# thuanz123/enhancing-transformers

Hardware: AMD Instinct MI355X
Metric: images/sec ViT-VQGAN-base 256px stage-1 train; VQ argmin match-rate (higher is better)
Workload: dtype fp16; 1 GPU; imagenet_vitvq_base.yaml AE training step (1 fwd + 1 bwd + grad all-reduce + AdamW), loss = 1.0*L2 + 1.0*codebook (LPIPS/GAN weights 0), K=8192 x 32 l2-normalised codes, fp32 master weights, fp16 MFMA operands / fp32 accumulate, dynamic loss scale (now 65536; device-side inf/nan step skip + GradScaler update rule); per_gpu_batch=128, global_batch=128, image=256x256, parallelism=dp1, hip_graph_replay=False

## Files before the change

### enhancing-transformers_amd/csrc/common.h

```cpp
#pragma once
#include <hip/hip_runtime.h>
#include <stdint.h>
#include <stdio.h>
#include "../../include/enh_hip.h"

#define LDS_AS __attribute__((address_space(3)))
#define GLB_AS __attribute__((address_space(1)))
#ifdef ENH_GLDS_AUX_OVERRIDE
#define ENH_GLDS_AUX ENH_GLDS_AUX_OVERRIDE
#else
#define ENH_GLDS_AUX 0
#endif

typedef __attribute__((ext_vector_type(4))) float f32x4;
typedef __attribute__((ext_vector_type(4))) unsigned int u32x4;
typedef __attribute__((ext_vector_type(2))) unsigned int u32x2;
typedef __attribute__((ext_vector_type(16))) float f32x16;
typedef __attribute__((ext_vector_type(8))) __bf16 bf16x8;
typedef __attribute__((ext_vector_type(8))) short s16x8;
typedef __attribute__((ext_vector_type(4))) short s16x4;
typedef __attribute__((__vector_size__(4 * sizeof(__bf16)))) __bf16 bf16x4_t;

void enh_set_error(const char* fmt, ...);
int enh_check_launch(const char* what);
// ... 49 lines not shown
  else return (float)__builtin_bit_cast(f16x2_t, u)[1];
}
template <typename OT>
__device__ inline float unpack1(uint16_t h) {
  if constexpr (OT::id == 0) return __builtin_bit_cast(float, (uint32_t)h << 16);
  else return (float)__builtin_bit_cast(_Float16, h);
}
template <typename OT>
__device__ inline uint16_t pack1(float f) {
  if constexpr (OT::id == 0) return f32_to_bf16_bits(f);
  else return __builtin_bit_cast(uint16_t, (_Float16)f);
}
template <typename OT>
__device__ __forceinline__ f32x16 mfma32(const s16x8& a, const s16x8& b, const f32x16& c) {
  if constexpr (OT::id == 0) return __builtin_amdgcn_mfma_f32_32x32x16_bf16(__builtin_bit_cast(bf16x8, a), __builtin_bit_cast(bf16x8, b), c, 0, 0, 0);
  else return __builtin_amdgcn_mfma_f32_32x32x16_f16(__builtin_bit_cast(f16x8, a), __builtin_bit_cast(f16x8, b), c, 0, 0, 0);
}
template <typename OT>
__device__ __forceinline__ f32x4 mfma16(const s16x8& a, const s16x8& b, const f32x4& c) {
  if constexpr (OT::id == 0) return __builtin_amdgcn_mfma_f32_16x16x32_bf16(__builtin_bit_cast(bf16x8, a), __builtin_bit_cast(bf16x8, b), c, 0, 0, 0);
  else return __builtin_amdgcn_mfma_f32_16x16x32_f16(__builtin_bit_cast(f16x8, a), __builtin_bit_cast(f16x8, b), c, 0, 0, 0);
}
#define ENH_DT_DISPATCH(dtype, CALL)                    \
  do {                                                   \
    if ((dtype) == ENH_DT_F16) { typedef F16 OT; CALL; } \
    else { typedef BF16 OT; CALL; }                      \
  } while (0)
#define ENH_REQUIRE_DT(dtype, what) ENH_REQUIRE((dtype) == ENH_DT_BF16 || (dtype) == ENH_DT_F16, ENH_E_BADARG, what ": dtype must be ENH_DT_BF16 (0) or ENH_DT_F16 (1), got %d", (int)(dtype))

__device__ __forceinline__ float tanh_x3(float x) {
  const float x2 = x * x;
  const float t = __builtin_amdgcn_exp2f(x * 2.8853900817779268f);
  const float big = 1.f - 2.f * __builtin_amdgcn_rcpf(t + 1.f);
  const float small = x * (1.f + x2 * (-0.33333333333f + x2 * (0.13333333333f + x2 * -0.05396825397f)));
  return x2 < 0.0144f ? small : big;
}

__device__ inline s16x4 lds_tr_read_b64(const void* lds_ptr) {
  bf16x4_t v = __builtin_amdgcn_ds_read_tr16_b64_v4bf16((LDS_AS bf16x4_t*)lds_ptr);
  return __builtin_bit_cast(s16x4, v);
}

__device__ inline void lds_tr_read_b64_asm(unsigned long long& out, const void* lds_ptr) {
  const unsigned addr = (unsigned)(uintptr_t)(LDS_AS const void*)lds_ptr;
  asm volatile("ds_read_b64_tr_b16 %0, %1" : "=v"(out) : "v"(addr) : "memory");
}

__device__ inline float wave_sum(float v) {
#pragma unroll
  for (int o = 32; o > 0; o >>= 1) v += __shfl_xor(v, o, 64);
  return v;
}

__device__ inline float fixed_order_rowsum16(const float* __restrict__ part, int rows, int64_t stride, int64_t n, bool n_ok, float* s_red ) {
  const int col = threadIdx.x & 15, grp = threadIdx.x >> 4;
  const int per = (rows + 15) / 16;
  const int r0 = grp * per, r1 = r0 + per < rows ? r0 + per : rows;
  float a = 0.f;
  if (n_ok)
    for (int r = r0; r < r1; ++r) a += part[(int64_t)r * stride + n];
  s_red[grp * 16 + col] = a;
  __syncthreads();
  float t = 0.f;
  if (grp == 0)
    for (int g = 0; g < 16; ++g) t += s_red[g * 16 + col];
  return t;
}
```

### enhancing-transformers_amd/csrc/elementwise.hip

```cpp
#include "common.h"

template <typename OT>
__global__ void patchify_kernel(const float* __restrict__ img, int B, int C, int H, int W, int p,
                                uint16_t* __restrict__ out, int64_t total4) {
  const int64_t i = (int64_t)blockIdx.x * blockDim.x + threadIdx.x;
  if (i >= total4) return;
  const int p4 = p >> 2, gx_n = W / p, gy_n = H / p;
  int64_t r = i;
  const int q = (int)(r % p4); r /= p4;
  const int ph = (int)(r % p); r /= p;
  const int c = (int)(r % C); r /= C;
  const int gx = (int)(r % gx_n);
  const int gy = (int)((r / gx_n) % gy_n);
  const int b = (int)(r / ((int64_t)gx_n * gy_n));
  const float4 v = *reinterpret_cast<const float4*>(img + (((size_t)b * C + c) * H + (size_t)gy * p + ph) * W + (size_t)gx * p + q * 4);
  *reinterpret_cast<uint2*>(out + (size_t)i * 4) = make_uint2(pack2<OT>(v.x, v.y), pack2<OT>(v.z, v.w));
}

template <typename OT>
__global__ __launch_bounds__(256) void unpatchify_loss_kernel(
    const float* __restrict__ pix, const float* __restrict__ target, int B, int C, int H, int W, int p, float w_l1,
    float w_l2, float inv_numel, float* __restrict__ xrec, double* __restrict__ sums, uint16_t* __restrict__ dpix,
    int64_t total4, const float* __restrict__ gscale) {
  __shared__ float s_l1[4], s_l2[4];
  if (gscale) inv_numel *= *gscale;
  const int64_t i = (int64_t)blockIdx.x * blockDim.x + threadIdx.x;
  float l1 = 0.f, l2 = 0.f;
  if (i < total4) {
    const int p4 = p >> 2, gx_n = W / p, gy_n = H / p;
    int64_t r = i;
    const int q = (int)(r % p4); r /= p4;
    const int ph = (int)(r % p); r /= p;
    const int c = (int)(r % C); r /= C;
    const int gx = (int)(r % gx_n);
    const int gy = (int)((r / gx_n) % gy_n);
    const int b = (int)(r / ((int64_t)gx_n * gy_n));
    const size_t off = (((size_t)b * C + c) * H + (size_t)gy * p + ph) * W + (size_t)gx * p + q * 4;
    const float4 v = *reinterpret_cast<const float4*>(pix + (size_t)i * 4);
    if (xrec) *reinterpret_cast<float4*>(xrec + off) = v;
    if (target) {
      const float4 x = *reinterpret_cast<const float4*>(target + off);
      const float d[4] = {v.x - x.x, v.y - x.y, v.z - x.z, v.w - x.w};
      float g[4];
#pragma unroll
      for (int k = 0; k < 4; ++k) {
        l1 += fabsf(d[k]);
        l2 += d[k] * d[k];
        const float sg = d[k] > 0.f ? 1.f : (d[k] < 0.f ? -1.f : 0.f);
        g[k] = (w_l1 * sg + w_l2 * 2.f * d[k]) * inv_numel;
      }
      if (dpix) *reinterpret_cast<uint2*>(dpix + (size_t)i * 4) = make_uint2(pack2<OT>(g[0], g[1]), pack2<OT>(g[2], g[3]));
    }
  }
  if (sums) {
    l1 = wave_sum(l1);
    l2 = wave_sum(l2);
    if ((threadIdx.x & 63) == 0) { s_l1[threadIdx.x >> 6] = l1; s_l2[threadIdx.x >> 6] = l2; }
    __syncthreads();
    if (threadIdx.x == 0) {
      atomicAdd(&sums[0], (double)((s_l1[0] + s_l1[1]) + (s_l1[2] + s_l1[3])));
      atomicAdd(&sums[1], (double)((s_l2[0] + s_l2[1]) + (s_l2[2] + s_l2[3])));
    }
  }
}

template <typename OT>
__global__ __launch_bounds__(256) void colsum_h16_kernel(const uint16_t* __restrict__ x, int64_t M, int64_t N,
                                                          int64_t ldx, int64_t rows_per_block, float* __restrict__ out, int64_t part_stride) {
  __shared__ float s_part[3][128];
  const int lane = threadIdx.x & 63, wave = threadIdx.x >> 6;
  const int64_t n0 = (int64_t)blockIdx.x * 128 + lane * 2;
  const int64_t m_begin = (int64_t)blockIdx.y * rows_per_block;
  int64_t m_end = m_begin + rows_per_block;
  if (m_end > M) m_end = M;
  float a0 = 0.f, a1 = 0.f;
  if (n0 < N) {
    for (int64_t m = m_begin + wave; m < m_end; m += 4) {
      const uint32_t u = *reinterpret_cast<const uint32_t*>(x + (size_t)m * ldx + n0);
      a0 += unpack_lo<OT>(u);
      a1 += unpack_hi<OT>(u);
    }
  }
  if (wave > 0) { s_part[wave - 1][lane * 2] = a0; s_part[wave - 1][lane * 2 + 1] = a1; }
  __syncthreads();
  if (wave == 0 && n0 < N) {
    for (int ww = 0; ww < 3; ++ww) { a0 += s_part[ww][lane * 2]; a1 += s_part[ww][lane * 2 + 1]; }
    { if (part_stride) out[(int64_t)blockIdx.y * part_stride + n0] = a0; else atomicAdd(&out[n0], a0); }
    { if (part_stride) out[(int64_t)blockIdx.y * part_stride + n0 + 1] = a1; else atomicAdd(&out[n0 + 1], a1); }
  }
}

template <typename OT>
__global__ __launch_bounds__(256) void colsum_h16_wide_kernel(const uint16_t* __restrict__ x, int64_t M, int64_t N, int64_t ldx,
                                                               int64_t rows_per_block, float* __restrict__ out, int64_t part_stride) {
  __shared__ float s_part[3][512];
  const int lane = threadIdx.x & 63, wave = threadIdx.x >> 6;
  const int64_t n0 = (int64_t)blockIdx.x * 512 + lane * 8;
  const int64_t m_begin = (int64_t)blockIdx.y * rows_per_block;
  int64_t m_end = m_begin + rows_per_block;
  if (m_end > M) m_end = M;
  float acc[8] = {0.f, 0.f, 0.f, 0.f, 0.f, 0.f, 0.f, 0.f};
  if (n0 < N) {
    const uint16_t* col = x + n0;
    int64_t m = m_begin + wave;
    for (; m + 12 < m_end; m += 16) {
      u32x4 v[4];
#pragma unroll
      for (int r = 0; r < 4; ++r) v[r] = *reinterpret_cast<const u32x4*>(col + (size_t)(m + 4 * r) * ldx);
#pragma unroll
      for (int r = 0; r < 4; ++r)
#pragma unroll
        for (int k = 0; k < 4; ++k) {
          acc[2 * k] += unpack_lo<OT>(v[r][k]);
          acc[2 * k + 1] += unpack_hi<OT>(v[r][k]);
        }
// ... 42 lines not shown
  if (i >= n) return;
  if (skip && *skip != 0.f) return;
  if (loss_scale) gscale /= *loss_scale;
  float pv[4], gv[4], mv[4], vv[4];
  const bool full = i + 3 < n;
  if (full) {
    const float4 a = *reinterpret_cast<const float4*>(p + i), b = *reinterpret_cast<const float4*>(g + i);
    const float4 c = *reinterpret_cast<const float4*>(m + i), d = *reinterpret_cast<const float4*>(v + i);
    pv[0] = a.x; pv[1] = a.y; pv[2] = a.z; pv[3] = a.w; gv[0] = b.x; gv[1] = b.y; gv[2] = b.z; gv[3] = b.w;
    mv[0] = c.x; mv[1] = c.y; mv[2] = c.z; mv[3] = c.w; vv[0] = d.x; vv[1] = d.y; vv[2] = d.z; vv[3] = d.w;
  } else {
    for (int k = 0; k < 4; ++k) {
      const bool ok = i + k < n;
      pv[k] = ok ? p[i + k] : 0.f; gv[k] = ok ? g[i + k] : 0.f; mv[k] = ok ? m[i + k] : 0.f; vv[k] = ok ? v[i + k] : 0.f;
    }
  }
#pragma unroll
  for (int k = 0; k < 4; ++k) {
    const float gg = gv[k] * gscale;
    pv[k] = pv[k] * (1.0f - lr * wd);
    mv[k] = mv[k] * beta1 + gg * (1.0f - beta1);
    vv[k] = vv[k] * beta2 + gg * gg * (1.0f - beta2);
    const float denom = sqrtf(vv[k]) * inv_sqrt_bc2 + eps;
    pv[k] = pv[k] - (lr * inv_bc1) * (mv[k] / denom);
  }
  if (full) {
    *reinterpret_cast<float4*>(p + i) = make_float4(pv[0], pv[1], pv[2], pv[3]);
    *reinterpret_cast<float4*>(m + i) = make_float4(mv[0], mv[1], mv[2], mv[3]);
    *reinterpret_cast<float4*>(v + i) = make_float4(vv[0], vv[1], vv[2], vv[3]);
    if (p16) *reinterpret_cast<uint2*>(p16 + i) = make_uint2(pack2<OT>(pv[0], pv[1]), pack2<OT>(pv[2], pv[3]));
  } else {
    for (int k = 0; k < 4 && i + k < n; ++k) {
      p[i + k] = pv[k]; m[i + k] = mv[k]; v[i + k] = vv[k];
      if (p16) p16[i + k] = pack1<OT>(pv[k]);
    }
  }
}

extern "C" int enh_patchify(const float* img, int B, int C, int H, int W, int p, enh_h16* patches, int dtype, void* stream) {
  ENH_REQUIRE_DT(dtype, "enh_patchify");
  ENH_REQUIRE(img && patches, ENH_E_BADARG, "enh_patchify: null pointer");
  ENH_REQUIRE(B > 0 && C > 0 && p > 0 && p % 4 == 0 && H % p == 0 && W % p == 0, ENH_E_SHAPE, "enh_patchify: need p %% 4 == 0 and H,W divisible by p (B=%d C=%d H=%d W=%d p=%d)", B, C, H, W, p);
  const int64_t total4 = (int64_t)B * C * H * W / 4;
  ENH_DT_DISPATCH(dtype, (patchify_kernel<OT><<<(int)((total4 + 255) / 256), 256, 0, (hipStream_t)stream>>>(img, B, C, H, W, p, patches, total4)));
  return enh_check_launch("enh_patchify");
}

extern "C" int enh_unpatchify_loss(const float* pix, const float* target, int B, int C, int H, int W, int p, float w_l1,
                                   float w_l2, float* xrec, double* sums, enh_h16* dpix_bf16, const float* grad_scale_dev, int dtype, void* stream) {
  ENH_REQUIRE_DT(dtype, "enh_unpatchify_loss");
  ENH_REQUIRE(pix && (xrec || target), ENH_E_BADARG, "enh_unpatchify_loss: null pointer");
  ENH_REQUIRE(B > 0 && C > 0 && p > 0 && p % 4 == 0 && H % p == 0 && W % p == 0, ENH_E_SHAPE, "enh_unpatchify_loss: need p %% 4 == 0 and H,W divisible by p");
  const int64_t numel = (int64_t)B * C * H * W, total4 = numel / 4;
  ENH_DT_DISPATCH(dtype, (unpatchify_loss_kernel<OT><<<(int)((total4 + 255) / 256), 256, 0, (hipStream_t)stream>>>(
      pix, target, B, C, H, W, p, w_l1, w_l2, 1.0f / (float)numel, xrec, target ? sums : nullptr, dpix_bf16, total4, grad_scale_dev)));
  return enh_check_launch("enh_unpatchify_loss");
}

__global__ __launch_bounds__(256) void colsum_reduce_kernel(const float* __restrict__ part, int chunks, int64_t N, float* __restrict__ out, int accumulate) {
  __shared__ float s_red[256];
  const int64_t n = (int64_t)blockIdx.x * 16 + (threadIdx.x & 15);
  const float t = fixed_order_rowsum16(part, chunks, N, n, n < N, s_red);
  if ((threadIdx.x >> 4) == 0 && n < N) out[n] = accumulate ? out[n] + t : t;
}

int enh_colsum_reduce_launch(const float* part, int chunks, int64_t N, float* out, int accumulate, hipStream_t s) {
  colsum_reduce_kernel<<<dim3((unsigned)((N + 15) / 16)), 256, 0, s>>>(part, chunks, N, out, accumulate);
  return enh_check_launch("colsum_reduce");
}

static int64_t colsum_chunks(int64_t M) {
  const int64_t chunks = (M + 511) / 512;
  return chunks > 256 ? 256 : chunks;
}

extern "C" size_t enh_colsum_h16_workspace_bytes(int64_t M, int64_t N) { return M > 0 && N > 0 ? (size_t)colsum_chunks(M) * N * sizeof(float) : 0; }

static int colsum_h16_impl(const enh_h16* x, int64_t M, int64_t N, int64_t ldx, float* out, int accumulate, float* part, int dtype, void* stream) {
  ENH_REQUIRE_DT(dtype, "enh_colsum_h16");
  ENH_REQUIRE(x && out, ENH_E_BADARG, "enh_colsum_h16: null pointer");
  ENH_REQUIRE(M > 0 && N > 0 && N % 2 == 0 && ldx % 2 == 0, ENH_E_SHAPE, "enh_colsum_h16: N and ldx must be even");
  hipStream_t s = (hipStream_t)stream;
  if (!accumulate && !part) {
    const int rc = enh_zero_f32_launch(out, N, s);
    if (rc) return rc;
  }
  const int64_t chunks = colsum_chunks(M);
  const int64_t rows_per_block = (M + chunks - 1) / chunks;
  float* dst = part ? part : out;
  const int64_t stride = part ? N : 0;
  if (N % 8 == 0 && ldx % 8 == 0 && ((uintptr_t)x & 15) == 0) {
    dim3 grid((unsigned)((N + 511) / 512), (unsigned)chunks);
    ENH_DT_DISPATCH(dtype, (colsum_h16_wide_kernel<OT><<<grid, 256, 0, s>>>(x, M, N, ldx, rows_per_block, dst, stride)));
  } else {
    dim3 grid((unsigned)((N + 127) / 128), (unsigned)chunks);
    ENH_DT_DISPATCH(dtype, (colsum_h16_kernel<OT><<<grid, 256, 0, s>>>(x, M, N, ldx, rows_per_block, dst, stride)));
  }
  if (part) colsum_reduce_kernel<<<dim3((unsigned)((N + 15) / 16)), 256, 0, s>>>(part, (int)chunks, N, out, accumulate);
  return enh_check_launch("enh_colsum_h16");
}

extern "C" int enh_colsum_h16(const enh_h16* x, int64_t M, int64_t N, int64_t ldx, float* out, int accumulate, int dtype, void* stream) {
  return colsum_h16_impl(x, M, N, ldx, out, accumulate, nullptr, dtype, stream);
}

extern "C" int enh_colsum_h16_ws(const enh_h16* x, int64_t M, int64_t N, int64_t ldx, float* out, int accumulate, void* ws, size_t ws_bytes, int dtype, void* stream) {
  ENH_REQUIRE(ws && ws_bytes >= enh_colsum_h16_workspace_bytes(M, N), ENH_E_WORKSPACE, "enh_colsum_h16_ws: workspace too small (%zu bytes)", ws_bytes);
  return colsum_h16_impl(x, M, N, ldx, out, accumulate, (float*)ws, dtype, stream);
}

template <typename OT>
__global__ void cast_f32_h16_head_scaled_kernel(const float* __restrict__ x, uint16_t* __restrict__ y, int64_t n, int64_t n_scaled, float alpha,
                                                 int64_t x_stride, int64_t y_stride) {
  x += (int64_t)blockIdx.y * x_stride; y += (int64_t)blockIdx.y * y_stride;
  const int64_t i = ((int64_t)blockIdx.x * blockDim.x + threadIdx.x) * 4;
  if (i >= n) return;
  if (i + 3 < n) {
    float4 v = *reinterpret_cast<const float4*>(x + i);
    if (i < n_scaled) { v.x *= alpha; v.y *= alpha; v.z *= alpha; v.w *= alpha; }
    *reinterpret_cast<uint2*>(y + i) = make_uint2(pack2<OT>(v.x, v.y), pack2<OT>(v.z, v.w));
  } else {
    for (int64_t k = i; k < n; ++k) y[k] = pack1<OT>(x[k] * (k < n_scaled ? alpha : 1.0f));
  }
}

extern "C" int enh_cast_f32_h16_head_scaled(const float* x, enh_h16* y, int64_t n, int64_t n_scaled, float alpha, int dtype, void* stream) {
  ENH_REQUIRE_DT(dtype, "enh_cast_f32_h16_head_scaled");
  ENH_REQUIRE(x && y && n > 0 && n_scaled >= 0 && n_scaled <= n && n_scaled % 4 == 0, ENH_E_BADARG, "enh_cast_f32_h16_head_scaled: bad argument");
  const int64_t n4 = (n + 3) / 4;
  ENH_DT_DISPATCH(dtype, (cast_f32_h16_head_scaled_kernel<OT><<<(int)((n4 + 255) / 256), 256, 0, (hipStream_t)stream>>>(x, y, n, n_scaled, alpha, 0, 0)));
  return enh_check_launch("enh_cast_f32_h16_head_scaled");
}

extern "C" int enh_cast_f32_h16_head_scaled_strided(const float* x, int64_t x_stride, enh_h16* y, int64_t y_stride, int64_t n, int64_t n_scaled, float alpha,
                                                     int count, int dtype, void* stream) {
  ENH_REQUIRE_DT(dtype, "enh_cast_f32_h16_head_scaled_strided");
  ENH_REQUIRE(x && y && n > 0 && n_scaled >= 0 && n_scaled <= n && n_scaled % 4 == 0 && count > 0 && count <= 65535, ENH_E_BADARG,
              "enh_cast_f32_h16_head_scaled_strided: bad argument");
  ENH_REQUIRE(x_stride % 4 == 0 && y_stride % 4 == 0 && y_stride >= n, ENH_E_SHAPE, "enh_cast_f32_h16_head_scaled_strided: strides must be multiples of 4 elements and the outputs disjoint");
  const int64_t n4 = (n + 3) / 4;
  ENH_DT_DISPATCH(dtype, (cast_f32_h16_head_scaled_kernel<OT><<<dim3((unsigned)((n4 + 255) / 256), (unsigned)count), 256, 0, (hipStream_t)stream>>>(x, y, n, n_scaled, alpha, x_stride, y_stride)));
  return enh_check_launch("enh_cast_f32_h16_head_scaled_strided");
}

extern "C" int enh_cast_f32_h16(const float* x, enh_h16* y, int64_t n, int dtype, void* stream) {
  ENH_REQUIRE_DT(dtype, "enh_cast_f32_h16");
  ENH_REQUIRE(x && y && n > 0, ENH_E_BADARG, "enh_cast_f32_h16: bad argument");
  const int64_t n4 = (n + 3) / 4;
  ENH_DT_DISPATCH(dtype, (cast_f32_h16_kernel<OT><<<(int)((n4 + 255) / 256), 256, 0, (hipStream_t)stream>>>(x, y, n)));
  return enh_check_launch("enh_cast_f32_h16");
}
// ... 77 lines not shown
```

### enhancing-transformers_amd/csrc/layernorm.hip

```cpp
#include "common.h"

template <int NCH, bool X3, typename OT>
__global__ __launch_bounds__(256) void ln_fwd_kernel(const float* __restrict__ x, const float* __restrict__ w,
                                                     const float* __restrict__ b, int64_t M, int D, float eps,
                                                     uint16_t* __restrict__ y16, float* __restrict__ y32,
                                                     float* __restrict__ mean_out, float* __restrict__ rstd_out, uint16_t* __restrict__ y3) {
  const int lane = threadIdx.x & 63;
  const int64_t row = (int64_t)blockIdx.x * 4 + (threadIdx.x >> 6);
  if (row >= M) return;
  const int nch = D >> 2;
  const float4* xr = reinterpret_cast<const float4*>(x + (size_t)row * D);
  float4 v[NCH];
  float s = 0.f;
#pragma unroll
  for (int i = 0; i < NCH; ++i) {
    const int c = lane + 64 * i;
    v[i] = c < nch ? xr[c] : make_float4(0.f, 0.f, 0.f, 0.f);
    s += (v[i].x + v[i].y) + (v[i].z + v[i].w);
  }
  const float mean = wave_sum(s) / (float)D;
  float q = 0.f;
#pragma unroll
  for (int i = 0; i < NCH; ++i) {
    const int c = lane + 64 * i;
// ... 179 lines not shown
            for (int ww = 0; ww < 3; ++ww) ax[k] += s_dw[ww][c * 4 + k];
            if (part) part[((size_t)blockIdx.x * 3 + 2) * D + c * 4 + k] = ax[k];
            else atomicAdd(&dxsum[c * 4 + k], ax[k]);
          }
        }
      }
    }
  }
}

template <bool X3, typename OT>
static void ln_fwd_launch(int grid, hipStream_t s, const float* x, const float* w, const float* b, int64_t M, int D, float eps, enh_h16* y_bf16, float* y_f32,
                          float* mean, float* rstd, enh_h16* y3) {
  switch ((D + 255) / 256) {
    case 1: ln_fwd_kernel<1, X3, OT><<<grid, 256, 0, s>>>(x, w, b, M, D, eps, y_bf16, y_f32, mean, rstd, y3); break;
    case 2: ln_fwd_kernel<2, X3, OT><<<grid, 256, 0, s>>>(x, w, b, M, D, eps, y_bf16, y_f32, mean, rstd, y3); break;
    case 3: ln_fwd_kernel<3, X3, OT><<<grid, 256, 0, s>>>(x, w, b, M, D, eps, y_bf16, y_f32, mean, rstd, y3); break;
    case 4: ln_fwd_kernel<4, X3, OT><<<grid, 256, 0, s>>>(x, w, b, M, D, eps, y_bf16, y_f32, mean, rstd, y3); break;
    case 5: ln_fwd_kernel<5, X3, OT><<<grid, 256, 0, s>>>(x, w, b, M, D, eps, y_bf16, y_f32, mean, rstd, y3); break;
    default: ln_fwd_kernel<8, X3, OT><<<grid, 256, 0, s>>>(x, w, b, M, D, eps, y_bf16, y_f32, mean, rstd, y3); break;
  }
}

extern "C" int enh_layernorm_forward(const float* x, const float* w, const float* b, int64_t M, int D, float eps,
                                     enh_h16* y_bf16, float* y_f32, float* mean, float* rstd, int dtype, void* stream) {
  ENH_REQUIRE_DT(dtype, "enh_layernorm_forward");
  ENH_REQUIRE(x && w && b && (y_bf16 || y_f32), ENH_E_BADARG, "enh_layernorm_forward: null pointer");
  ENH_REQUIRE(M > 0 && D > 0 && D % 4 == 0 && D <= 2048, ENH_E_SHAPE, "enh_layernorm_forward: need D %% 4 == 0 and D <= 2048, got M=%lld D=%d", (long long)M, D);
  ENH_DT_DISPATCH(dtype, (ln_fwd_launch<false, OT>((int)((M + 3) / 4), (hipStream_t)stream, x, w, b, M, D, eps, y_bf16, y_f32, mean, rstd, nullptr)));
  return enh_check_launch("enh_layernorm_forward");
}

extern "C" int enh_layernorm_forward_x3(const float* x, const float* w, const float* b, int64_t M, int D, float eps, enh_h16* y3,
                                        enh_h16* y_bf16, float* y_f32, float* mean, float* rstd, void* stream) {
  ENH_REQUIRE(x && w && b && y3, ENH_E_BADARG, "enh_layernorm_forward_x3: null pointer");
  ENH_REQUIRE(M > 0 && D > 0 && D % 4 == 0 && D <= 2048, ENH_E_SHAPE, "enh_layernorm_forward_x3: need D %% 4 == 0 and D <= 2048, got M=%lld D=%d", (long long)M, D);
  ln_fwd_launch<true, BF16>((int)((M + 3) / 4), (hipStream_t)stream, x, w, b, M, D, eps, y_bf16, y_f32, mean, rstd, y3);
  return enh_check_launch("enh_layernorm_forward_x3");
}

template <bool DY16, typename OT>
static void ln_bwd_launch(int grid, hipStream_t s, const void* dy, const float* x, const float* w, const float* mean, const float* rstd,
                          const float* dres, int64_t M, int D, float* dx_f32, enh_h16* dx_bf16, float* dw, float* db, float* dx_colsum, float* part) {
  switch ((D + 255) / 256) {
    case 1: ln_bwd_kernel<1, DY16, OT><<<grid, 256, 0, s>>>(dy, x, w, mean, rstd, dres, M, D, dx_f32, dx_bf16, dw, db, dx_colsum, part); break;
    case 2: ln_bwd_kernel<2, DY16, OT><<<grid, 256, 0, s>>>(dy, x, w, mean, rstd, dres, M, D, dx_f32, dx_bf16, dw, db, dx_colsum, part); break;
    case 3: ln_bwd_kernel<3, DY16, OT><<<grid, 256, 0, s>>>(dy, x, w, mean, rstd, dres, M, D, dx_f32, dx_bf16, dw, db, dx_colsum, part); break;
    case 4: ln_bwd_kernel<4, DY16, OT><<<grid, 256, 0, s>>>(dy, x, w, mean, rstd, dres, M, D, dx_f32, dx_bf16, dw, db, dx_colsum, part); break;
    case 5: ln_bwd_kernel<5, DY16, OT><<<grid, 256, 0, s>>>(dy, x, w, mean, rstd, dres, M, D, dx_f32, dx_bf16, dw, db, dx_colsum, part); break;
    default: ln_bwd_kernel<8, DY16, OT><<<grid, 256, 0, s>>>(dy, x, w, mean, rstd, dres, M, D, dx_f32, dx_bf16, dw, db, dx_colsum, part); break;
  }
}

__global__ __launch_bounds__(256) void ln_bwd_reduce_kernel(const float* __restrict__ part, int nwg, int D, float* __restrict__ dw, float* __restrict__ db,
                                                            float* __restrict__ dxsum) {
  __shared__ float s_red[256];
  const int which = blockIdx.y;
  float* out = which == 0 ? dw : (which == 1 ? db : dxsum);
  if (!out) return;
  const int j = blockIdx.x * 16 + (threadIdx.x & 15);
  const float t = fixed_order_rowsum16(part + (size_t)which * D, nwg, (int64_t)3 * D, j, j < D, s_red);
  if ((threadIdx.x >> 4) == 0 && j < D) out[j] += t;
}

static int ln_bwd_grid(int64_t M, bool for_workspace = false) {
  const int64_t want = (M + 3) / 4;
  const int cus = for_workspace ? enh_device_cus() : enh_cu_budget();
  return (int)(want < cus ? want : cus);
}

extern "C" size_t enh_layernorm_backward_workspace_bytes(int64_t M, int D) {
  return M > 0 && D > 0 ? (size_t)ln_bwd_grid(M, true) * 3 * D * sizeof(float) : 0;
}

static int ln_bwd_impl(const float* dy, const enh_h16* dy_bf16, const float* x, const float* w, const float* mean, const float* rstd, const float* dres,
                       int64_t M, int D, float* dx_f32, enh_h16* dx_bf16, float* dw, float* db, float* dx_colsum, float* part, int dtype, void* stream) {
  ENH_REQUIRE_DT(dtype, "enh_layernorm_backward");
  ENH_REQUIRE((dy != nullptr) != (dy_bf16 != nullptr), ENH_E_BADARG, "enh_layernorm_backward: pass exactly one of dy (f32) / dy_bf16");
  ENH_REQUIRE(x && w && mean && rstd && dx_f32 && dw && db, ENH_E_BADARG, "enh_layernorm_backward: null pointer");
  ENH_REQUIRE(M > 0 && D > 0 && D % 4 == 0 && D <= 2048, ENH_E_SHAPE, "enh_layernorm_backward: need D %% 4 == 0 and D <= 2048, got M=%lld D=%d", (long long)M, D);
  hipStream_t s = (hipStream_t)stream;
  const int grid = ln_bwd_grid(M);
  if (dy_bf16) ENH_DT_DISPATCH(dtype, (ln_bwd_launch<true, OT>(grid, s, dy_bf16, x, w, mean, rstd, dres, M, D, dx_f32, dx_bf16, dw, db, dx_colsum, part)));
  else ENH_DT_DISPATCH(dtype, (ln_bwd_launch<false, OT>(grid, s, dy, x, w, mean, rstd, dres, M, D, dx_f32, dx_bf16, dw, db, dx_colsum, part)));
  if (part) ln_bwd_reduce_kernel<<<dim3((unsigned)((D + 15) / 16), 3), 256, 0, s>>>(part, grid, D, dw, db, dx_colsum);
  return enh_check_launch("enh_layernorm_backward");
}

extern "C" int enh_layernorm_backward(const float* dy, const enh_h16* dy_bf16, const float* x, const float* w, const float* mean,
                                      const float* rstd, const float* dres, int64_t M, int D, float* dx_f32,
                                      enh_h16* dx_bf16, float* dw, float* db, float* dx_colsum, int dtype, void* stream) {
  return ln_bwd_impl(dy, dy_bf16, x, w, mean, rstd, dres, M, D, dx_f32, dx_bf16, dw, db, dx_colsum, nullptr, dtype, stream);
}

extern "C" int enh_layernorm_backward_ws(const float* dy, const enh_h16* dy_bf16, const float* x, const float* w, const float* mean,
                                         const float* rstd, const float* dres, int64_t M, int D, float* dx_f32,
                                         enh_h16* dx_bf16, float* dw, float* db, float* dx_colsum, void* ws, size_t ws_bytes, int dtype, void* stream) {
  ENH_REQUIRE(ws && ws_bytes >= enh_layernorm_backward_workspace_bytes(M, D), ENH_E_WORKSPACE, "enh_layernorm_backward_ws: workspace too small (%zu bytes)", ws_bytes);
  return ln_bwd_impl(dy, dy_bf16, x, w, mean, rstd, dres, M, D, dx_f32, dx_bf16, dw, db, dx_colsum, (float*)ws, dtype, stream);
}
```

### enhancing-transformers_amd/csrc/vq.hip

```cpp
#include "common.h"

#define VQ_D 32
#define VQ_TILE 128
#define VQ_PITCH 36
#define VQ_MAXD 8

__device__ inline float chain16_sq(const float* x) {
  float s = 0.f;
#pragma unroll
  for (int j = 0; j < 16; ++j) s = fmaf(x[j], x[j], s);
  return s;
}

__device__ __forceinline__ void vq_load16(float (&x)[16], const float* __restrict__ row, int off, int d) {
#pragma unroll
  for (int q = 0; q < 4; ++q) {
    const float4 v = off + 4 * q < d ? *reinterpret_cast<const float4*>(row + off + 4 * q) : make_float4(0.f, 0.f, 0.f, 0.f);
    x[q * 4 + 0] = v.x; x[q * 4 + 1] = v.y; x[q * 4 + 2] = v.z; x[q * 4 + 3] = v.w;
  }
}
__device__ __forceinline__ void vq_store16(float* __restrict__ row, const float (&o)[16], int off, int d) {
#pragma unroll
  for (int q = 0; q < 4; ++q)
    if (off + 4 * q < d) *reinterpret_cast<float4*>(row + off + 4 * q) = make_float4(o[q * 4], o[q * 4 + 1], o[q * 4 + 2], o[q * 4 + 3]);
// ... 368 lines not shown
  }

  if (live) {
#pragma unroll
    for (int c = 0; c < NC; ++c) {
      float z0[16], acc[16], o[16];
      vq_load16(z0, zrow, off0 + c * 16, d);
#pragma unroll
      for (int j = 0; j < 16; ++j) acc[j] = 0.f;
#pragma unroll
      for (int i = 0; i < VQ_MAXD; ++i) {
        if (i < depth) {
          const float4* ep = reinterpret_cast<const float4*>(en + (size_t)code[i] * DW + off0 + c * 16);
#pragma unroll
          for (int q = 0; q < 4; ++q) {
            const float4 v = ep[q];
            acc[q * 4 + 0] = acc[q * 4 + 0] + v.x; acc[q * 4 + 1] = acc[q * 4 + 1] + v.y;
            acc[q * 4 + 2] = acc[q * 4 + 2] + v.z; acc[q * 4 + 3] = acc[q * 4 + 3] + v.w;
          }
        }
      }
#pragma unroll
      for (int j = 0; j < 16; ++j) o[j] = z0[j] + (acc[j] - z0[j]);
      vq_store16(zq_out + (size_t)tok * d, o, off0 + c * 16, d);
      if (zq_bf16) vq_store16_h(zq_bf16 + (size_t)tok * d, o, off0 + c * 16, d, f16);
    }
  }
}

__global__ void vq_loss_finalize_kernel(const float* __restrict__ partials, int nblocks, int depth, int64_t M, int d,
                                        float beta, float* __restrict__ loss_out) {
  __shared__ double s_acc[256];
  float total = 0.f;
  for (int dpt = 0; dpt < depth; ++dpt) {
    double a = 0.0;
    for (int b = threadIdx.x; b < nblocks; b += blockDim.x) a += (double)partials[(size_t)b * depth + dpt];
    s_acc[threadIdx.x] = a;
    __syncthreads();
    for (int o = 128; o > 0; o >>= 1) {
      if ((int)threadIdx.x < o) s_acc[threadIdx.x] += s_acc[threadIdx.x + o];
      __syncthreads();
    }
    if (threadIdx.x == 0) {
      const float m = (float)(s_acc[0] / ((double)M * d));
      total += beta * m + m;
    }
    __syncthreads();
  }
  if (threadIdx.x == 0) loss_out[0] = total / (float)depth;
}

#define VQ_CPW 32
#define VQ_RS 16
__global__ __launch_bounds__(256) void vq_de_partial_kernel(const int* __restrict__ codes, const float* __restrict__ contrib, int64_t n, int K,
                                                            int d, float* __restrict__ part) {
  __shared__ int s_list[256];
  __shared__ int s_wc[4];
  __shared__ float s_acc[8][VQ_CPW][VQ_D];
  const int t = threadIdx.x, lane = t & 63, wave = t >> 6, grp = t >> 5, gl = t & 31;
  const int cb = blockIdx.x * VQ_CPW, slice = blockIdx.y;
  const int dc = blockIdx.z * VQ_D + gl;
  const bool cv = dc < d;
  const int64_t per = ((n + (int64_t)VQ_RS * 256 - 1) / ((int64_t)VQ_RS * 256)) * 256;
  const int64_t e0 = (int64_t)slice * per, e1 = e0 + per < n ? e0 + per : n;
#pragma unroll
  for (int k = 0; k < 8 * VQ_CPW * VQ_D / 256; ++k) (&s_acc[0][0][0])[t + 256 * k] = 0.f;
  for (int64_t base = e0; base < e1; base += 256) {
    const int64_t e = base + t;
    const unsigned lc = e < e1 ? (unsigned)(codes[e] - cb) : 0xffffffffu;
    const bool hit = lc < (unsigned)VQ_CPW;
    const unsigned long long m = __ballot(hit);
    if (lane == 0) s_wc[wave] = __popcll(m);
    __syncthreads();
    int off = 0, total = 0;
#pragma unroll
    for (int w = 0; w < 4; ++w) { const int c = s_wc[w]; if (w < wave) off += c; total += c; }
    if (hit) s_list[off + __popcll(m & ((1ull << lane) - 1ull))] = t | ((int)lc << 8);
    __syncthreads();
    for (int q0 = grp; q0 < total; q0 += 32) {
      float v[4];
      int c[4];
#pragma unroll
      for (int u = 0; u < 4; ++u) {
        const int q = q0 + 8 * u;
        c[u] = -1;
        v[u] = 0.f;
        if (q < total) {
          const int item = s_list[q];
          c[u] = item >> 8;
          v[u] = cv ? contrib[(size_t)(base + (item & 255)) * d + dc] : 0.f;
        }
      }
#pragma unroll
      for (int u = 0; u < 4; ++u)
        if (c[u] >= 0) s_acc[grp][c[u]][gl] += v[u];
    }
  }
  __syncthreads();
#pragma unroll
  for (int k = 0; k < VQ_CPW * VQ_D / 256; ++k) {
    const int idx = t + 256 * k, c = idx >> 5, col = idx & 31;
    float a = s_acc[0][c][col];
#pragma unroll
    for (int g = 1; g < 8; ++g) a += s_acc[g][c][col];
    const int oc = blockIdx.z * VQ_D + col;
    if (cb + c < K && oc < d) part[((size_t)slice * K + cb + c) * d + oc] = a;
  }
}
__global__ __launch_bounds__(256) void vq_de_finalize_kernel(const float* __restrict__ part, int K, int d, float* __restrict__ dE) {
  const int64_t i = (int64_t)blockIdx.x * 256 + threadIdx.x;
  if (i >= (int64_t)K * d) return;
  float s = part[i];
#pragma unroll
  for (int r = 1; r < VQ_RS; ++r) s += part[(size_t)r * K * d + i];
  dE[i] += s;
}

template <int MAXD, int DW>
__global__ __launch_bounds__(256) void vq_bwd_kernel(
    const float* __restrict__ z, const float* __restrict__ E, const float* __restrict__ en,
    const float* __restrict__ enrm, const int64_t* __restrict__ idx, const float* __restrict__ g_out, float g_loss,
    const float* __restrict__ g_loss_dev, int64_t M, int d, int depth, int use_norm, int use_residual, float beta,
    float* __restrict__ dz, uint16_t* __restrict__ dz_bf16, int f16, float* __restrict__ contrib, int* __restrict__ codes) {
  constexpr int P = DW / 16, TPW = 64 / P;
  const int lane = threadIdx.x & 63;
  const int col = lane & (TPW - 1), hi = lane / TPW;
  const int off = hi * 16;
  const int64_t tok = ((int64_t)blockIdx.x * (blockDim.x >> 6) + (threadIdx.x >> 6)) * TPW + col;
  const bool live = tok < M;
  const int64_t tk = live ? tok : 0;
  float gL = g_loss * (g_loss_dev ? g_loss_dev[0] : 1.f) / (float)depth;
  const float c = 2.0f / ((float)M * (float)d);

  float r[16], zn[MAXD][16], e[MAXD][16], den[MAXD];
  int code[MAXD];
  vq_load16(r, z + (size_t)tk * d, off, d);
#pragma unroll
  for (int i = 0; i < MAXD; ++i) {
    if (i < depth) {
      if (use_norm) {
        float sp = chain16_sq(r);
        float s = vq_tok_sum<P>(sp);
        den[i] = fmaxf(sqrtf(s), 1e-12f);
      } else den[i] = 1.f;
#pragma unroll
      for (int j = 0; j < 16; ++j) zn[i][j] = use_norm ? r[j] / den[i] : r[j];
      code[i] = (int)idx[(size_t)tk * depth + i];
      const float4* ep = reinterpret_cast<const float4*>(en + (size_t)code[i] * DW + off);
// ... 218 lines not shown
```

Before: 630.6 images/s.

## Tile unpatchify loss via LDS, widen column reductions, batch VQ code scans

Adds an LDS-tiled unpatchify+loss kernel that stages image tiles in shared memory, so target reads and xrec writes are coalesced in image layout rather than strided per patch. It also widens the fixed-order column-sum reductions to 32 columns per block, with batched unrolled loads for more memory-level parallelism. The VQ codebook-gradient scatter now scans 8 chunks of 256 codes per pair of barriers, cutting synchronisation per code. Risks include more LDS use and a fallback path only for shapes that fail the tiling checks.

```diff
diff --git a/enhancing-transformers_amd/csrc/common.h b/enhancing-transformers_amd/csrc/common.h
--- a/enhancing-transformers_amd/csrc/common.h
+++ b/enhancing-transformers_amd/csrc/common.h
@@ -125,17 +125,32 @@
   return v;
 }
 
+#define ROWSUM16_COLS 32
+#define ROWSUM16_THREADS (16 * ROWSUM16_COLS)
+template <int U>
+__device__ __forceinline__ float rowsum_batch(const float* __restrict__ p, int64_t stride, float a) {
+  float v[U];
+#pragma unroll
+  for (int u = 0; u < U; ++u) v[u] = p[(int64_t)u * stride];
+#pragma unroll
+  for (int u = 0; u < U; ++u) a += v[u];
+  return a;
+}
 __device__ inline float fixed_order_rowsum16(const float* __restrict__ part, int rows, int64_t stride, int64_t n, bool n_ok, float* s_red ) {
-  const int col = threadIdx.x & 15, grp = threadIdx.x >> 4;
+  const int col = threadIdx.x & (ROWSUM16_COLS - 1), grp = threadIdx.x / ROWSUM16_COLS;
   const int per = (rows + 15) / 16;
   const int r0 = grp * per, r1 = r0 + per < rows ? r0 + per : rows;
   float a = 0.f;
-  if (n_ok)
-    for (int r = r0; r < r1; ++r) a += part[(int64_t)r * stride + n];
-  s_red[grp * 16 + col] = a;
+  if (n_ok) {
+    int r = r0;
+    for (; r + 32 <= r1; r += 32) a = rowsum_batch<32>(part + (int64_t)r * stride + n, stride, a);
+    if (r + 16 <= r1) { a = rowsum_batch<16>(part + (int64_t)r * stride + n, stride, a); r += 16; }
+    for (; r < r1; ++r) a += part[(int64_t)r * stride + n];
+  }
+  s_red[grp * ROWSUM16_COLS + col] = a;
   __syncthreads();
   float t = 0.f;
   if (grp == 0)
-    for (int g = 0; g < 16; ++g) t += s_red[g * 16 + col];
+    for (int g = 0; g < 16; ++g) t += s_red[g * ROWSUM16_COLS + col];
   return t;
 }
diff --git a/enhancing-transformers_amd/csrc/elementwise.hip b/enhancing-transformers_amd/csrc/elementwise.hip
--- a/enhancing-transformers_amd/csrc/elementwise.hip
+++ b/enhancing-transformers_amd/csrc/elementwise.hip
@@ -15,6 +15,20 @@
   const int b = (int)(r / ((int64_t)gx_n * gy_n));
   const float4 v = *reinterpret_cast<const float4*>(img + (((size_t)b * C + c) * H + (size_t)gy * p + ph) * W + (size_t)gx * p + q * 4);
   *reinterpret_cast<uint2*>(out + (size_t)i * 4) = make_uint2(pack2<OT>(v.x, v.y), pack2<OT>(v.z, v.w));
+}
+
+template <typename OT>
+__device__ __forceinline__ uint2 pixel_loss_quad(const float4& v, const float4& x, float w_l1, float w_l2, float inv_numel, float& l1, float& l2) {
+  const float d[4] = {v.x - x.x, v.y - x.y, v.z - x.z, v.w - x.w};
+  float g[4];
+#pragma unroll
+  for (int k = 0; k < 4; ++k) {
+    l1 += fabsf(d[k]);
+    l2 += d[k] * d[k];
+    const float sg = d[k] > 0.f ? 1.f : (d[k] < 0.f ? -1.f : 0.f);
+    g[k] = (w_l1 * sg + w_l2 * 2.f * d[k]) * inv_numel;
+  }
+  return make_uint2(pack2<OT>(g[0], g[1]), pack2<OT>(g[2], g[3]));
 }
 
 template <typename OT>
@@ -39,17 +53,8 @@
     const float4 v = *reinterpret_cast<const float4*>(pix + (size_t)i * 4);
     if (xrec) *reinterpret_cast<float4*>(xrec + off) = v;
     if (target) {
-      const float4 x = *reinterpret_cast<const float4*>(target + off);
-      const float d[4] = {v.x - x.x, v.y - x.y, v.z - x.z, v.w - x.w};
-      float g[4];
-#pragma unroll
-      for (int k = 0; k < 4; ++k) {
-        l1 += fabsf(d[k]);
-        l2 += d[k] * d[k];
-        const float sg = d[k] > 0.f ? 1.f : (d[k] < 0.f ? -1.f : 0.f);
-        g[k] = (w_l1 * sg + w_l2 * 2.f * d[k]) * inv_numel;
-      }
-      if (dpix) *reinterpret_cast<uint2*>(dpix + (size_t)i * 4) = make_uint2(pack2<OT>(g[0], g[1]), pack2<OT>(g[2], g[3]));
+      const uint2 g = pixel_loss_quad<OT>(v, *reinterpret_cast<const float4*>(target + off), w_l1, w_l2, inv_numel, l1, l2);
+      if (dpix) *reinterpret_cast<uint2*>(dpix + (size_t)i * 4) = g;
     }
   }
   if (sums) {
@@ -61,6 +66,99 @@
       atomicAdd(&sums[0], (double)((s_l1[0] + s_l1[1]) + (s_l1[2] + s_l1[3])));
       atomicAdd(&sums[1], (double)((s_l2[0] + s_l2[1]) + (s_l2[2] + s_l2[3])));
     }
+  }
+}
+
+#define UNP_TILE_FLOATS 4096
+#define UNP_PAD_FLOATS 256
+template <typename OT, int NP>
+__global__ __launch_bounds__(256) void unpatchify_loss_tiled_kernel(
+    const float* __restrict__ pix, const float* __restrict__ target, int C, int H, int W, int p, int G, float w_l1, float w_l2, float inv_numel,
+    float* __restrict__ xrec, double* __restrict__ sums, uint16_t* __restrict__ dpix, int ntiles, const float* __restrict__ gscale) {
+  __shared__ __attribute__((aligned(16))) float s_tile[UNP_TILE_FLOATS + UNP_PAD_FLOATS];
+  __shared__ float s_l1[NP][4], s_l2[NP][4];
+  if (gscale) inv_numel *= *gscale;
+  const int t = threadIdx.x;
+  const int cpp = C * p * p, ps = cpp + p, qpr = G * p / 4;
+  const int gy_n = H / p, cpr = (W / p) / G;
+  int lds_img[NP], off_img[NP], lds_pix[NP];
+#pragma unroll
+  for (int k = 0; k < NP; ++k) {
+    const int j = t + 256 * k;
+    const int row = j / qpr, x = (j - row * qpr) * 4;
+    const int c = row / p, ph = row - c * p, gl = x / p;
+    lds_img[k] = gl * ps + row * p + (x - gl * p);
+    off_img[k] = (c * H + ph) * W + x;
+    lds_pix[k] = 4 * j + (4 * j / cpp) * p;
+  }
+  double acc1 = 0.0, acc2 = 0.0;
+  for (int tl = blockIdx.x; tl < ntiles; tl += gridDim.x) {
+    const int prow = tl / cpr, gc = tl - prow * cpr;
+    const int b = prow / gy_n, gy = prow - b * gy_n;
+    const size_t ibase = ((size_t)b * C * H + (size_t)gy * p) * W + (size_t)gc * G * p;
+    const size_t pbase = (size_t)tl * (NP * 1024) + (size_t)t * 4;
+    float4 v[NP];
+#pragma unroll
+    for (int k = 0; k < NP; ++k) v[k] = *reinterpret_cast<const float4*>(pix + pbase + 1024 * k);
+    if (target) {
+      float4 x[NP];
+#pragma unroll
+      for (int k = 0; k < NP; ++k) x[k] = *reinterpret_cast<const float4*>(target + ibase + off_img[k]);
+#pragma unroll
+      for (int k = 0; k < NP; ++k) *reinterpret_cast<float4*>(&s_tile[lds_img[k]]) = x[k];
+      __syncthreads();
+#pragma unroll
+      for (int k = 0; k < NP; ++k) {
+        float l1 = 0.f, l2 = 0.f;
+        const uint2 g = pixel_loss_quad<OT>(v[k], *reinterpret_cast<const float4*>(&s_tile[lds_pix[k]]), w_l1, w_l2, inv_numel, l1, l2);
+        if (dpix) *reinterpret_cast<uint2*>(dpix + pbase + 1024 * k) = g;
+        if (sums) {
+          l1 = wave_sum(l1);
+          l2 = wave_sum(l2);
+          if ((t & 63) == 0) { s_l1[k][t >> 6] = l1; s_l2[k][t >> 6] = l2; }
+        }
+      }
+    }
+    if (xrec) {
+#pragma unroll
+      for (int k = 0; k < NP; ++k) *reinterpret_cast<float4*>(&s_tile[lds_pix[k]]) = v[k];
+    }
+    __syncthreads();
+    if (xrec) {
+#pragma unroll
+      for (int k = 0; k < NP; ++k) *reinterpret_cast<float4*>(xrec + ibase + off_img[k]) = *reinterpret_cast<const float4*>(&s_tile[lds_img[k]]);
+    }
+    if (sums && t == 0) {
+#pragma unroll
+      for (int k = 0; k < NP; ++k) {
+        acc1 += (double)((s_l1[k][0] + s_l1[k][1]) + (s_l1[k][2] + s_l1[k][3]));
+        acc2 += (double)((s_l2[k][0] + s_l2[k][1]) + (s_l2[k][2] + s_l2[k][3]));
+      }
+    }
+    __syncthreads();
+  }
+  if (sums && t == 0) {
+    atomicAdd(&sums[0], acc1);
+    atomicAdd(&sums[1], acc2);
+  }
+}
+
+static int unpatchify_tile_patches(int64_t B, int C, int H, int W, int p) {
+  const int64_t cpp = (int64_t)C * p * p;
+  if ((int64_t)C * H * W >= INT32_MAX || B * (H / p) * (W / p) >= INT32_MAX) return 0;
+  for (int G = W / p; G >= 1; --G)
+    if ((W / p) % G == 0 && G * cpp <= UNP_TILE_FLOATS && (G * cpp) % 1024 == 0 && G * p >= 32 && G * p <= UNP_PAD_FLOATS) return G;
+  return 0;
+}
+
+template <typename OT>
+static void unpatchify_loss_tiled_launch(int np, int grid, hipStream_t s, const float* pix, const float* target, int C, int H, int W, int p, int G, float w_l1,
+                                         float w_l2, float inv_numel, float* xrec, double* sums, uint16_t* dpix, int ntiles, const float* gscale) {
+  switch (np) {
+    case 1: unpatchify_loss_tiled_kernel<OT, 1><<<grid, 256, 0, s>>>(pix, target, C, H, W, p, G, w_l1, w_l2, inv_numel, xrec, sums, dpix, ntiles, gscale); break;
+    case 2: unpatchify_loss_tiled_kernel<OT, 2><<<grid, 256, 0, s>>>(pix, target, C, H, W, p, G, w_l1, w_l2, inv_numel, xrec, sums, dpix, ntiles, gscale); break;
+    case 3: unpatchify_loss_tiled_kernel<OT, 3><<<grid, 256, 0, s>>>(pix, target, C, H, W, p, G, w_l1, w_l2, inv_numel, xrec, sums, dpix, ntiles, gscale); break;
+    default: unpatchify_loss_tiled_kernel<OT, 4><<<grid, 256, 0, s>>>(pix, target, C, H, W, p, G, w_l1, w_l2, inv_numel, xrec, sums, dpix, ntiles, gscale); break;
   }
 }
 
@@ -209,20 +307,30 @@
   ENH_REQUIRE(pix && (xrec || target), ENH_E_BADARG, "enh_unpatchify_loss: null pointer");
   ENH_REQUIRE(B > 0 && C > 0 && p > 0 && p % 4 == 0 && H % p == 0 && W % p == 0, ENH_E_SHAPE, "enh_unpatchify_loss: need p %% 4 == 0 and H,W divisible by p");
   const int64_t numel = (int64_t)B * C * H * W, total4 = numel / 4;
-  ENH_DT_DISPATCH(dtype, (unpatchify_loss_kernel<OT><<<(int)((total4 + 255) / 256), 256, 0, (hipStream_t)stream>>>(
-      pix, target, B, C, H, W, p, w_l1, w_l2, 1.0f / (float)numel, xrec, target ? sums : nullptr, dpix_bf16, total4, grad_scale_dev)));
+  double* sums_used = target ? sums : nullptr;
+  const int G = unpatchify_tile_patches(B, C, H, W, p);
+  if (G) {
+    const int ntiles = (int)((int64_t)B * (H / p) * (W / p) / G), np = (int)((int64_t)G * C * p * p / 1024);
+    const int fill = 8 * enh_cu_budget();
+    ENH_DT_DISPATCH(dtype, (unpatchify_loss_tiled_launch<OT>(np, ntiles < fill ? ntiles : fill, (hipStream_t)stream, pix, target, C, H, W, p, G, w_l1, w_l2,
+                                                             1.0f / (float)numel, xrec, sums_used, dpix_bf16, ntiles, grad_scale_dev)));
+  } else {
+    ENH_DT_DISPATCH(dtype, (unpatchify_loss_kernel<OT><<<(int)((total4 + 255) / 256), 256, 0, (hipStream_t)stream>>>(
+        pix, target, B, C, H, W, p, w_l1, w_l2, 1.0f / (float)numel, xrec, sums_used, dpix_bf16, total4, grad_scale_dev)));
+  }
   return enh_check_launch("enh_unpatchify_loss");
 }
 
-__global__ __launch_bounds__(256) void colsum_reduce_kernel(const float* __restrict__ part, int chunks, int64_t N, float* __restrict__ out, int accumulate) {
-  __shared__ float s_red[256];
-  const int64_t n = (int64_t)blockIdx.x * 16 + (threadIdx.x & 15);
+__global__ __launch_bounds__(ROWSUM16_THREADS) void colsum_reduce_kernel(const float* __restrict__ part, int chunks, int64_t N, float* __restrict__ out,
+                                                                         int accumulate) {
+  __shared__ float s_red[ROWSUM16_THREADS];
+  const int64_t n = (int64_t)blockIdx.x * ROWSUM16_COLS + (threadIdx.x & (ROWSUM16_COLS - 1));
   const float t = fixed_order_rowsum16(part, chunks, N, n, n < N, s_red);
-  if ((threadIdx.x >> 4) == 0 && n < N) out[n] = accumulate ? out[n] + t : t;
+  if (threadIdx.x < ROWSUM16_COLS && n < N) out[n] = accumulate ? out[n] + t : t;
 }
 
 int enh_colsum_reduce_launch(const float* part, int chunks, int64_t N, float* out, int accumulate, hipStream_t s) {
-  colsum_reduce_kernel<<<dim3((unsigned)((N + 15) / 16)), 256, 0, s>>>(part, chunks, N, out, accumulate);
+  colsum_reduce_kernel<<<dim3((unsigned)((N + ROWSUM16_COLS - 1) / ROWSUM16_COLS)), ROWSUM16_THREADS, 0, s>>>(part, chunks, N, out, accumulate);
   return enh_check_launch("colsum_reduce");
 }
 
@@ -253,7 +361,7 @@
     dim3 grid((unsigned)((N + 127) / 128), (unsigned)chunks);
     ENH_DT_DISPATCH(dtype, (colsum_h16_kernel<OT><<<grid, 256, 0, s>>>(x, M, N, ldx, rows_per_block, dst, stride)));
   }
-  if (part) colsum_reduce_kernel<<<dim3((unsigned)((N + 15) / 16)), 256, 0, s>>>(part, (int)chunks, N, out, accumulate);
+  if (part) colsum_reduce_kernel<<<dim3((unsigned)((N + ROWSUM16_COLS - 1) / ROWSUM16_COLS)), ROWSUM16_THREADS, 0, s>>>(part, (int)chunks, N, out, accumulate);
   return enh_check_launch("enh_colsum_h16");
 }
 
diff --git a/enhancing-transformers_amd/csrc/layernorm.hip b/enhancing-transformers_amd/csrc/layernorm.hip
--- a/enhancing-transformers_amd/csrc/layernorm.hip
+++ b/enhancing-transformers_amd/csrc/layernorm.hip
@@ -255,15 +255,15 @@
   }
 }
 
-__global__ __launch_bounds__(256) void ln_bwd_reduce_kernel(const float* __restrict__ part, int nwg, int D, float* __restrict__ dw, float* __restrict__ db,
-                                                            float* __restrict__ dxsum) {
-  __shared__ float s_red[256];
+__global__ __launch_bounds__(ROWSUM16_THREADS) void ln_bwd_reduce_kernel(const float* __restrict__ part, int nwg, int D, float* __restrict__ dw,
+                                                                         float* __restrict__ db, float* __restrict__ dxsum) {
+  __shared__ float s_red[ROWSUM16_THREADS];
   const int which = blockIdx.y;
   float* out = which == 0 ? dw : (which == 1 ? db : dxsum);
   if (!out) return;
-  const int j = blockIdx.x * 16 + (threadIdx.x & 15);
+  const int j = blockIdx.x * ROWSUM16_COLS + (threadIdx.x & (ROWSUM16_COLS - 1));
   const float t = fixed_order_rowsum16(part + (size_t)which * D, nwg, (int64_t)3 * D, j, j < D, s_red);
-  if ((threadIdx.x >> 4) == 0 && j < D) out[j] += t;
+  if (threadIdx.x < ROWSUM16_COLS && j < D) out[j] += t;
 }
 
 static int ln_bwd_grid(int64_t M, bool for_workspace = false) {
@@ -286,7 +286,7 @@
   const int grid = ln_bwd_grid(M);
   if (dy_bf16) ENH_DT_DISPATCH(dtype, (ln_bwd_launch<true, OT>(grid, s, dy_bf16, x, w, mean, rstd, dres, M, D, dx_f32, dx_bf16, dw, db, dx_colsum, part)));
   else ENH_DT_DISPATCH(dtype, (ln_bwd_launch<false, OT>(grid, s, dy, x, w, mean, rstd, dres, M, D, dx_f32, dx_bf16, dw, db, dx_colsum, part)));
-  if (part) ln_bwd_reduce_kernel<<<dim3((unsigned)((D + 15) / 16), 3), 256, 0, s>>>(part, grid, D, dw, db, dx_colsum);
+  if (part) ln_bwd_reduce_kernel<<<dim3((unsigned)((D + ROWSUM16_COLS - 1) / ROWSUM16_COLS), 3), ROWSUM16_THREADS, 0, s>>>(part, grid, D, dw, db, dx_colsum);
   return enh_check_launch("enh_layernorm_backward");
 }
 
diff --git a/enhancing-transformers_amd/csrc/vq.hip b/enhancing-transformers_amd/csrc/vq.hip
--- a/enhancing-transformers_amd/csrc/vq.hip
+++ b/enhancing-transformers_amd/csrc/vq.hip
@@ -444,10 +444,11 @@
 
 #define VQ_CPW 32
 #define VQ_RS 16
+#define VQ_SCAN 8
 __global__ __launch_bounds__(256) void vq_de_partial_kernel(const int* __restrict__ codes, const float* __restrict__ contrib, int64_t n, int K,
                                                             int d, float* __restrict__ part) {
-  __shared__ int s_list[256];
-  __shared__ int s_wc[4];
+  __shared__ unsigned short s_list[VQ_SCAN][256];
+  __shared__ int s_wc[VQ_SCAN][4];
   __shared__ float s_acc[8][VQ_CPW][VQ_D];
   const int t = threadIdx.x, lane = t & 63, wave = t >> 6, grp = t >> 5, gl = t & 31;
   const int cb = blockIdx.x * VQ_CPW, slice = blockIdx.y;
@@ -457,35 +458,51 @@
   const int64_t e0 = (int64_t)slice * per, e1 = e0 + per < n ? e0 + per : n;
 #pragma unroll
   for (int k = 0; k < 8 * VQ_CPW * VQ_D / 256; ++k) (&s_acc[0][0][0])[t + 256 * k] = 0.f;
-  for (int64_t base = e0; base < e1; base += 256) {
-    const int64_t e = base + t;
-    const unsigned lc = e < e1 ? (unsigned)(codes[e] - cb) : 0xffffffffu;
-    const bool hit = lc < (unsigned)VQ_CPW;
-    const unsigned long long m = __ballot(hit);
-    if (lane == 0) s_wc[wave] = __popcll(m);
-    __syncthreads();
-    int off = 0, total = 0;
-#pragma unroll
-    for (int w = 0; w < 4; ++w) { const int c = s_wc[w]; if (w < wave) off += c; total += c; }
-    if (hit) s_list[off + __popcll(m & ((1ull << lane) - 1ull))] = t | ((int)lc << 8);
-    __syncthreads();
-    for (int q0 = grp; q0 < total; q0 += 32) {
-      float v[4];
-      int c[4];
-#pragma unroll
-      for (int u = 0; u < 4; ++u) {
-        const int q = q0 + 8 * u;
-        c[u] = -1;
-        v[u] = 0.f;
-        if (q < total) {
-          const int item = s_list[q];
-          c[u] = item >> 8;
-          v[u] = cv ? contrib[(size_t)(base + (item & 255)) * d + dc] : 0.f;
-        }
-      }
-#pragma unroll
-      for (int u = 0; u < 4; ++u)
-        if (c[u] >= 0) s_acc[grp][c[u]][gl] += v[u];
+  for (int64_t base = e0; base < e1; base += 256 * VQ_SCAN) {
+    unsigned lc[VQ_SCAN];
+#pragma unroll
+    for (int j = 0; j < VQ_SCAN; ++j) {
+      const int64_t e = base + 256 * j + t;
+      lc[j] = e < e1 ? (unsigned)(codes[e] - cb) : 0xffffffffu;
+    }
+    unsigned long long m[VQ_SCAN];
+#pragma unroll
+    for (int j = 0; j < VQ_SCAN; ++j) {
+      m[j] = __ballot(lc[j] < (unsigned)VQ_CPW);
+      if (lane == 0) s_wc[j][wave] = __popcll(m[j]);
+    }
+    __syncthreads();
+    int total[VQ_SCAN];
+#pragma unroll
+    for (int j = 0; j < VQ_SCAN; ++j) {
+      int off = 0;
+      total[j] = 0;
+#pragma unroll
+      for (int w = 0; w < 4; ++w) { const int c = s_wc[j][w]; if (w < wave) off += c; total[j] += c; }
+      if (lc[j] < (unsigned)VQ_CPW) s_list[j][off + __popcll(m[j] & ((1ull << lane) - 1ull))] = (unsigned short)(t | (lc[j] << 8));
+    }
+    __syncthreads();
+#pragma unroll
+    for (int j = 0; j < VQ_SCAN; ++j) {
+      const int64_t cbase = base + 256 * j;
+      for (int q0 = grp; q0 < total[j]; q0 += 32) {
+        float v[4];
+        int c[4];
+#pragma unroll
+        for (int u = 0; u < 4; ++u) {
+          const int q = q0 + 8 * u;
+          c[u] = -1;
+          v[u] = 0.f;
+          if (q < total[j]) {
+            const int item = s_list[j][q];
+            c[u] = item >> 8;
+            v[u] = cv ? contrib[(size_t)(cbase + (item & 255)) * d + dc] : 0.f;
+          }
+        }
+#pragma unroll
+        for (int u = 0; u < 4; ++u)
+          if (c[u] >= 0) s_acc[grp][c[u]][gl] += v[u];
+      }
     }
   }
   __syncthreads();
```

Measured after the change: 634.4 images/s, median of 6. Within noise of the previous version (+0.6%).
